# reonaledo/Multi-modality-Self-supervision

Measured on AMD Instinct MI355X. Metric: image-text pairs/sec pretraining step, BERT-base seq512, higher is better.
Workload: dtype f16

## Files before the change

### include/medvill_debug.h

```cpp
#ifndef MEDVILL_DEBUG_H_
#define MEDVILL_DEBUG_H_

#ifdef __cplusplus
extern "C" {
#endif

enum {
  MV_KNOB_ID_IMPL = 0,
  MV_KNOB_ID_GEMM_FORCE = 1,
  MV_KNOB_ID_GEMM_NJ = 2,
  MV_KNOB_ID_GEMM_DBG = 3,
  MV_KNOB_ID_ATTN_PLANES = 4,
  MV_KNOB_ID_PERSISTENT_CUS = 5,
  MV_KNOB_ID_ROWOPS_VARIANT = 6,
  MV_KNOB_ID_ATTN_FWD = 8,
  MV_KNOB_ID_GEMM_ROUNDS = 9,
  MV_KNOB_ID_ATTN_ORDER = 7
};
int mv_debug_set_knob(int id, int value);
int mv_debug_get_knob(int id);

#ifdef __cplusplus
}
#endif
#endif
```

### multi-modality-self-supervision_amd/_lib.py

```python
from __future__ import annotations

import ctypes as C
import os

import torch

HERE = os.path.dirname(os.path.abspath(__file__))
LIB_PATH = os.environ.get("MV_LIB_PATH") or os.path.join(HERE, "libmedvill_hip.so")
DBG_LIB_PATH = os.environ.get("MV_DBG_LIB_PATH") or (LIB_PATH[:-3] + "_dbg.so")

MV_F32, MV_BF16, MV_F16 = 0, 1, 2
EPI_NONE, EPI_BIAS, EPI_BIAS_GELU, EPI_BIAS_RES, EPI_DGELU, EPI_RES, EPI_BIAS_TANH, EPI_BIAS_GELU_D, EPI_MUL, EPI_BIAS_RELU, EPI_BIAS_RES_RELU = range(11)
_ERR = {-1: "MV_E_ARG (null pointer / bad size)", -2: "MV_E_SHAPE (unsupported shape or alignment)",
        -3: "MV_E_DTYPE", -4: "MV_E_WORKSPACE (workspace too small)", -5: "MV_E_NO_RCCL (librccl could not be loaded)"}

vp, i32, i64, f32, sz, u64, f64 = C.c_void_p, C.c_int, C.c_longlong, C.c_float, C.c_size_t, C.c_ulonglong, C.c_double

PROTOTYPES = {
    "mv_abi_version": [],
    "mv_build_info": [],
    "mv_stream_create_cumask": [vp, i32, C.POINTER(C.c_void_p)],
    "mv_stream_destroy": [vp],
    "mv_comm_unique_id": [vp],
    "mv_comm_init": [C.POINTER(C.c_void_p), i32, i32, vp],
# ... 53 lines not shown
    "mv_embed_rows": [i32, vp, vp, vp, vp, vp, vp, vp, vp, vp, i32, i32, i32, i32, i32, i32, f32, vp],
    "mv_ngram_ban": [vp, vp, i32, vp, vp, i32, i32, i32, vp, i32, vp, i32, vp, vp],
    "mv_logprob_topk_banned": [vp, i32, i32, i32, i32, i32, vp, i32, vp, vp, vp, vp, vp],
    "mv_bce_fwd_bwd": [vp, i32, vp, vp, i32, i32, vp, vp, i32, i32, vp, f32, vp, vp, vp, vp],
    "mv_rows_mul": [i32, vp, i32, vp, vp, i32, vp, i32, i32, vp, i32, vp],
    "mv_tensor_sqnorms": [vp, sz, vp, i32, vp, i32, vp, vp, vp],
    "mv_bce_multilabel": [vp, i32, vp, vp, i32, i32, vp, vp, i32, i32, vp, f32, vp, vp, vp, vp],
    "mv_bertadam_step": [vp, vp, vp, vp, vp, vp, sz, vp, i32, vp, i32, vp, f64, f64, f64, f32, f32, f32, i32, i32, f64, i32, vp, vp],
    "mv_lm_loss_fwd": [vp, i32, i32, i32, vp, vp, i32, f64, vp, vp, vp, vp],
    "mv_lm_loss_select": [vp, vp, vp, vp, i32, i32, i32, vp, vp, vp, vp],
    "mv_lm_loss_bwd": [vp, i32, i32, i32, vp, vp, vp, vp, i32, f64, vp, vp, vp, vp, vp, vp, i32, i32, vp],
    "mv_pair_draws": [u64, u64, i32, i32, vp, vp],
    "mv_pair_negatives": [vp, i32, i32, vp, u64, u64, vp, i32, vp, vp, vp],
    "mv_pair_assemble": [vp, vp, i32, vp, i32, i32, vp, vp, i32, i32, i32, i32, vp, vp, vp, vp, vp, vp, vp],
    "mv_rank_groups": [vp, vp, i32, i32, vp, i32, vp, vp, vp, vp, vp],
    "mv_report_draws": [u64, u64, i32, i32, vp, vp],
    "mv_report_assemble": [vp, vp, vp, i32, vp, i32, vp, vp, vp, i32, i32, i32, i32, i32, u64, u64, vp, vp, vp, vp, vp, vp, vp, vp, vp, vp],
    "mv_report_plan": [vp, vp, vp, vp, i32, i32, i32, i32, vp, vp, vp, vp, vp, vp, vp, vp],
    "mv_vqa_assemble": [vp, vp, vp, i32, vp, vp, vp, i32, vp, vp, i32, vp, i32, vp, vp, i32, i32, i32, i32, i32, vp, vp, vp, vp, vp, vp, vp, vp],
    "mv_vqa_score": [vp, vp, i32, i32, vp, vp, vp, i32, vp, vp, i32, vp, vp, vp],
    "mv_clf_assemble": [vp, vp, vp, vp, i32, vp, i32, vp, i32, vp, vp, i32, i32, i32, i32, i32, vp, vp, vp, vp, vp, vp, vp],
    "mv_clf_counts": [vp, i32, vp, i32, vp, i32, i32, vp, vp],
    "mv_bleu_words": [vp, i32, i32, i32, vp, vp, vp, i32, i64, i64, i64, vp, vp, vp],
    "mv_bleu_counts": [vp, i32, vp, i32, vp, i32, vp, i32, vp, vp, vp],
}
DEBUG_PROTOTYPES = {"mv_debug_set_knob": [i32, i32], "mv_debug_get_knob": [i32]}
_RESTYPE = {"mv_build_info": C.c_char_p, "mv_gemm_workspace_bytes": C.c_size_t, "mv_workspace_bytes": C.c_size_t,
            "mv_gemm_grouped_table_bytes": C.c_size_t, "mv_gemm_grouped_workspace_bytes": C.c_size_t}
ABI_VERSION = 6

KNOBS = {"impl": (0, 0), "gemm_force": (1, 0), "gemm_nj": (2, 0), "gemm_dbg": (3, 0), "attn_planes": (4, 16), "persistent_cus": (5, 0),
         "rowops_variant": (6, 0), "attn_order": (7, 0), "attn_fwd": (8, 0), "gemm_rounds": (9, 1)}

_lib = None
_dbg = None
_knobs = {k: d for k, (_, d) in KNOBS.items()}


def _open(path, protos):
    lib = C.CDLL(path)
    for name, args in protos.items():
        fn = getattr(lib, name)
        fn.argtypes = args
        fn.restype = _RESTYPE.get(name, C.c_int)
    if lib.mv_abi_version() != ABI_VERSION:
        raise RuntimeError(f"{path}: ABI version mismatch")
    return lib


def load(build_if_missing: bool = False):
    global _lib
    if _dbg is not None and any(_knobs[k] != d for k, (_, d) in KNOBS.items()):
        return _dbg
    if _lib is not None:
        return _lib
    if not os.path.exists(LIB_PATH):
        if build_if_missing:
            from ._build import build
            build()
        else:
            raise RuntimeError(
                f"{LIB_PATH} is missing: the gfx950 HIP extension has not been built. Run "
                "`python -c 'import __graft_entry__ as g; g.build()'` (needs hipcc). There is no fallback path.")
    _lib = _open(LIB_PATH, PROTOTYPES)
    return _lib


def set_knob(name: str, value: int):
    global _dbg
    kid, default = KNOBS[name]
    value = int(value)
    if _dbg is None:
        if value == default:
            return
        if not os.path.exists(DBG_LIB_PATH):
            raise RuntimeError(f"{DBG_LIB_PATH} is missing (the debug build of the library: __graft_entry__.build() makes both)")
        _dbg = _open(DBG_LIB_PATH, {**PROTOTYPES, **DEBUG_PROTOTYPES})
    check(_dbg.mv_debug_set_knob(kid, value), f"mv_debug_set_knob({name}, {value})")
    _knobs[name] = value


def get_knob(name: str) -> int:
    return _knobs[name]


def _knobs_from_env():
    spec = os.environ.get("MV_KNOBS", "")
    for item in filter(None, (x.strip() for x in spec.split(","))):
        k, _, v = item.partition("=")
        set_knob(k.strip(), int(v))


def check(rc: int, what: str):
    if rc == 0:
        return
    if rc <= -1000:
        raise RuntimeError(f"{what}: ncclResult_t {-1000 - rc}")
    if rc < 0:
        raise RuntimeError(f"{what}: {_ERR.get(rc, rc)}")
    raise RuntimeError(f"{what}: hipError_t {rc}")


def dt_of(t: torch.Tensor) -> int:
    if t.dtype == torch.float32:
        return MV_F32
    if t.dtype == torch.bfloat16:
        return MV_BF16
    if t.dtype == torch.float16:
        return MV_F16
    raise TypeError(f"unsupported dtype {t.dtype}")


def torch_dtype(dt: int):
    return {MV_F32: torch.float32, MV_BF16: torch.bfloat16, MV_F16: torch.float16}[dt]


# ... 16 lines not shown
```

### multi-modality-self-supervision_amd/csrc/mv_api.hip

```cpp
#include "mv_common.h"
#ifdef MV_DEBUG_KNOBS
#include "../../include/medvill_debug.h"
#endif

#define MV_KNOB_DEFAULTS {0, 0, 0, 0, 16, 0, 0, 0, 0, 1}
#ifdef MV_DEBUG_KNOBS
static int g_knobs[MV_KNOB_COUNT] = MV_KNOB_DEFAULTS;
int mv_knob(int id) { return g_knobs[id]; }
extern "C" int mv_debug_set_knob(int id, int value) {
  if (id < 0 || id >= MV_KNOB_COUNT) return MV_E_ARG;
  if (id == MV_KNOB_ATTN_PLANES && value != 8 && value != 12 && value != 16) return MV_E_ARG;
  g_knobs[id] = value;
  return MV_OK;
}
extern "C" int mv_debug_get_knob(int id) { return (id < 0 || id >= MV_KNOB_COUNT) ? MV_E_ARG : g_knobs[id]; }
#else
int mv_knob(int id) {
  static const int k[MV_KNOB_COUNT] = MV_KNOB_DEFAULTS;
  return k[id];
}
#endif

extern "C" int mv_abi_version(void) { return MV_ABI_VERSION; }
#ifdef MV_DEBUG_KNOBS
extern "C" const char* mv_build_info(void) { return "medvill-hip gfx950 debug-knobs (" __DATE__ " " __TIME__ ")"; }
#else
extern "C" const char* mv_build_info(void) { return "medvill-hip gfx950 (" __DATE__ " " __TIME__ ")"; }
#endif

extern "C" int mv_stream_create_cumask(const uint32_t* mask_words, int n_words, void** stream_out) {
  if (!mask_words || n_words <= 0 || !stream_out) return MV_E_ARG;
  hipStream_t st = nullptr;
  const hipError_t e = hipExtStreamCreateWithCUMask(&st, (uint32_t)n_words, mask_words);
  if (e != hipSuccess) return (int)e;
  *stream_out = (void*)st;
  return MV_OK;
}
extern "C" int mv_stream_destroy(void* stream) {
  if (!stream) return MV_E_ARG;
  const hipError_t e = hipStreamDestroy((hipStream_t)stream);
  return e == hipSuccess ? MV_OK : (int)e;
}
```

### multi-modality-self-supervision_amd/csrc/mv_attn.hip

```cpp
#include "mv_dispatch.h"

typedef float f32x2 __attribute__((ext_vector_type(2)));
#ifndef ATT_ABL
#define ATT_ABL 0
#endif
#ifndef ATT_EARLY_MASKS
#define ATT_EARLY_MASKS 0
#endif
#if ATT_ABL & 4096
__device__ unsigned long long g_att_prof[3][8];
__device__ unsigned long long g_att_tile[3][8];
#define PROF_DECL unsigned long long pt_ = clock64(), pacc_[6] = {0, 0, 0, 0, 0, 0}; unsigned long long ptile_[6] = {0, 0, 0, 0, 0, 0}
#define PROF_TILE_ARGS , unsigned long long (&ptile_)[6]
#define PROF_TILE_PASS , ptile_
#define PROF_T0 unsigned long long tt_ = clock64()
#define PROF_T(i, dep) do { asm volatile("s_nop 0" ::"v"(dep)); const unsigned long long n_ = clock64(); ptile_[i] += n_ - tt_; tt_ = n_; } while (0)
#define PROF_MARK(i) do { const unsigned long long n_ = clock64(); pacc_[i] += n_ - pt_; pt_ = n_; } while (0)
#define PROF_FLUSH(k) do { if (threadIdx.x == 0) { for (int i_ = 0; i_ < 6; ++i_) { atomicAdd(&g_att_prof[k][i_], pacc_[i_]); atomicAdd(&g_att_tile[k][i_], ptile_[i_]); } atomicAdd(&g_att_prof[k][7], 1ull); } } while (0)
#else
#define PROF_DECL
#define PROF_MARK(i)
#define PROF_FLUSH(k)
#define PROF_TILE_ARGS
#define PROF_TILE_PASS
// ... 187 lines not shown
      if (have == 0) { r = mv_hash32(base + ctr, k0, k1); ++ctr; have = PER; }
      const unsigned x = r & ((1u << SL) - 1u);
      r >>= SL;
      --have;
      if (x < lo) lt |= 1ull << l;
    }
  }
  out[w] = ~lt;
}

__device__ __forceinline__ int att_f(int r) { return (((r >> 1) & 1) << 2) | ((r >> 2) & 3); }
__device__ __forceinline__ int att_off(int r, int ch) { return r * 128 + ((ch ^ att_f(r)) << 4); }

__device__ __forceinline__ int acc_row(int reg, int h) { return (reg & 3) + 8 * (reg >> 2) + 4 * h; }

__device__ __forceinline__ void tile_load(u32x4 (&reg)[2], __amdgpu_buffer_rsrc_t rs, unsigned bytes, size_t rowbase,
                                          int row0, int nrows, int ld, int col0, int tid) {
#pragma unroll
  for (int i = 0; i < 2; ++i) {
    const int idx = tid + 256 * i;
    const int r = idx >> 3, ch = idx & 7;
    const bool ok = (row0 + r) < nrows;
    const unsigned off = (unsigned)(((rowbase + row0 + r) * (size_t)ld + col0 + ch * 8) * 2);
    reg[i] = __builtin_amdgcn_raw_buffer_load_b128(rs, ok ? off : bytes, 0, 0);
  }
}
__device__ __forceinline__ void tile_store(const u32x4 (&reg)[2], char* tile, int tid) {
#pragma unroll
  for (int i = 0; i < 2; ++i) {
    const int idx = tid + 256 * i;
    *(u32x4*)(tile + att_off(idx >> 3, idx & 7)) = reg[i];
  }
}
template <int NW>
__device__ __forceinline__ void tile_dma(dma_rsrc_t rs, unsigned bytes, size_t rowbase, int row0, int nrows, int ld,
                                         int col0, char* tile, int wid, int lane) {
#pragma unroll
  for (int i = 0; i < 8 / NW; ++i) {
    const int pc = wid + NW * i;
    const int r = pc * 8 + (lane >> 3), ch = (lane & 7) ^ att_f(r);
    const bool ok = (row0 + r) < nrows;
    const unsigned off = (unsigned)(((rowbase + row0 + r) * (size_t)ld + col0 + ch * 8) * 2);
    lds_dma16(rs, (MV_LDS void*)(tile + pc * 1024), ok ? off : bytes);
  }
}
#ifndef ATT_ISSUE_LATE
#define ATT_ISSUE_LATE 1
#endif
template <int N> __device__ __forceinline__ void att_wait_vmcnt() { asm volatile("s_waitcnt vmcnt(%0)" ::"n"(N) : "memory"); }
template <int PPW>
__device__ __forceinline__ void att_wait_stage(int younger) {
  if (younger <= 0) att_wait_vmcnt<0>();
  else if (younger == 1) att_wait_vmcnt<PPW>();
  else if (younger == 2) att_wait_vmcnt<2 * PPW>();
  else att_wait_vmcnt<3 * PPW>();
}

__device__ __forceinline__ bf16x8 frag_row(const char* tile, int base, int s, int l31, int h) {
  return *(const bf16x8*)(tile + att_off(base + l31, 2 * s + h));
}
__device__ __forceinline__ bf16x8 frag_tr(const char* tile, int cbase, int rb, int lane) {
  const int li = lane & 15, g = lane >> 4, h = g >> 1;
  const int col = cbase + 16 * (g & 1) + 4 * (li & 3);
  const int r = rb + 4 * h + (li >> 2);
  const int sub = (li & 1) * 8;
  bf16x4 lo = __builtin_amdgcn_ds_read_tr16_b64_v4bf16((MV_LDS bf16x4*)(tile + att_off(r, col >> 3) + sub));
  bf16x4 hi = __builtin_amdgcn_ds_read_tr16_b64_v4bf16((MV_LDS bf16x4*)(tile + att_off(r + 8, col >> 3) + sub));
  return __builtin_shufflevector(lo, hi, 0, 1, 2, 3, 4, 5, 6, 7);
}
struct FragLane { unsigned rk, tr; };
__device__ __forceinline__ FragLane frag_lane(int lane) {
// ... 345 lines not shown
        case 1: FWD_CALL(false, false); break;
        case 2: FWD_CALL(true, true); break;
        default: FWD_CALL(false, true); break;
      }
#undef FWD_CALL
    }
#if ATT_ABL & 4096
    asm volatile("s_nop 0" ::"v"(o[0][0]), "v"(o[1][15]));
#endif
    PROF_MARK(3);
    if (ATT_ISSUE_LATE && iss < nkt) issue();
    cur = next_tile(tmk.need, cur, nkt);
    ++done;
    PROF_MARK(4);
  }
  __builtin_amdgcn_s_barrier();
  const float ltot = lsum + __shfl_xor(lsum, 32, 64);
  const float inv = (a.drop_on ? a.inv_keep : 1.0f) / ltot;
  const int rows_ok = Lq - q0;
  char* patch = smem + wid * ATT_PATCH_BYTES;
  store_rows_tile<F16>(patch, o, inv, q_ok, a.out + (rowbase + q0) * (size_t)H + head * 64, (size_t)H, rows_ok, lane);
  if constexpr (F16) {
    if (a.out2) store_rows_tile<false>(patch, o, inv, q_ok, a.out2 + (rowbase + q0) * (size_t)H + head * 64, (size_t)H, rows_ok, lane);
  }
  if (q_ok && h == 0) a.lse[((size_t)b * a.A + head) * L + q] = (m2 + log2f(ltot)) * LN2;
#if ATT_ABL & 4096
  asm volatile("s_waitcnt vmcnt(0)");
#endif
  PROF_MARK(5);
  PROF_FLUSH(0);
}

template <bool MASKED, bool DROP, bool TAIL, bool F16>
__device__ __forceinline__ void dq_tile(const AttnArgs& a, unsigned tk, unsigned tv, unsigned tkt, const bf16x8 (&qf)[4], const bf16x8 (&dof)[4],
                                        f32x16 (&dq)[2], const uint32_t* myw, bool q_ok, int q, int b, int head, int k0, int Lv,
                                        float lse2, float dlt, float c2, int h, const unsigned long long* mp) {
  const float dlt_s = dlt * a.scale;
  const float dscale = DROP ? a.inv_keep * a.scale : a.scale;
#pragma unroll
  for (int kk = 0; kk < 2; ++kk) {
    f32x16 st, dp;
#pragma unroll
    for (int i = 0; i < 16; ++i) { st[i] = 0.f; dp[i] = 0.f; }
#pragma unroll
    for (int s = 0; s < 4; ++s) {
      st = mma32<F16>(frag_row_x(tk, 32 * kk, s), qf[s], st);
      dp = mma32<F16>(frag_row_x(tv, 32 * kk, s), dof[s], dp);
    }
    uint32_t w = 0xffffffffu;
    if (MASKED) { const int wi = (k0 >> 5) + kk; w = (q_ok && wi < a.W) ? myw[wi] : 0xffffffffu; }
    u64x8 m0, m1;
    if (DROP) sload_masks16(mp + 16 * kk, m0, m1);
#pragma unroll
    for (int r = 0; r < 16; ++r) {
      const int kr = acc_row(r, h);
      float pv;
      if (!MASKED) {
        pv = fexp2(fmaf(st[r], c2, -lse2));
      } else {
        const float v = fmaf(st[r], c2, ((w >> kr) & 1u) ? 0.f : MASK_ADD * LOG2E);
        pv = fexp2(v - lse2);
      }
      if (TAIL) pv = (k0 + 32 * kk + kr >= Lv) ? 0.f : pv;
      float t = fmaf(dp[r], dscale, -dlt_s);
      if (DROP) t = sel_set_else(t, -dlt_s, r < 8 ? m0[r & 7] : m1[r & 7]);
      st[r] = pv * t;
    }
#pragma unroll
    for (int s2 = 0; s2 < 2; ++s2) {
      const bf16x8 dsf = pack8t<F16>(st, s2);
#pragma unroll
      for (int dt = 0; dt < 2; ++dt)
        dq[dt] = mma32<F16>(frag_tr_x(tkt, dt, 32 * kk + 16 * s2), dsf, dq[dt]);
    }
  }
}

#define DQ_NS 4
template <bool F16>
__global__ __launch_bounds__(256, 2) void attn_bwd_dq_mfma_kernel(AttnArgs a) {
  extern __shared__ __attribute__((aligned(128))) char smem[];
  const int tid = threadIdx.x, lane = tid & 63, l31 = lane & 31, h = lane >> 5;
  const int wid = __builtin_amdgcn_readfirstlane(tid >> 6);
  int xb, head, b;
  att_block(a, xb, head, b);
  const int L = a.L, H = a.H, ld = 3 * a.H, T = a.T;
  const int qb0 = xb * 128, q0 = qb0 + wid * 32, q = q0 + l31;
  PROF_DECL;
  const TileMasks tmk = load_tile_masks_q(a.info, b, T, qb0 >> 6, min(q0 >> 6, T - 1), lane);
  const int Lv = a.cu ? a.cu[b + 1] - a.cu[b] : L;
  const int Lq = a.qlim ? min(Lv, a.qlim[b]) : Lv;
  if (qb0 >= Lv) return;
  const size_t rowbase = a.cu ? (size_t)a.cu[b] : (size_t)b * L;
  if (qb0 >= Lq) {
    const int r = qb0 + (tid >> 1);
    if (r < Lv) {
      bf16_t* z = a.dqkv + (rowbase + r) * (size_t)ld + head * 64 + 32 * (tid & 1);
#pragma unroll
      for (int c = 0; c < 32; c += 4) store4_16<F16>(z + c, 0.f, 0.f, 0.f, 0.f);
    }
    return;
  }
  const bool wave_on = q0 < Lq, q_ok = q < Lq;
  const size_t lrow = (size_t)b * L;
  __amdgpu_buffer_rsrc_t rs = __builtin_amdgcn_make_buffer_rsrc((void*)a.qkv, 0, a.bytes_qkv, 0x00020000);
  const dma_rsrc_t rsq = dma_rsrc(a.qkv, a.bytes_qkv);
  __amdgpu_buffer_rsrc_t rsd = __builtin_amdgcn_make_buffer_rsrc((void*)a.dctx, 0, a.bytes_ctx, 0x00020000);

  bf16x8 qf[4], dof[4];
#pragma unroll
  for (int s = 0; s < 4; ++s) {
    qf[s] = load_rowfrag_global(rs, a.bytes_qkv, rowbase + q, q_ok, ld, head * 64 + 16 * s + 8 * h);
    dof[s] = load_rowfrag_global(rsd, a.bytes_ctx, rowbase + q, q_ok, H, head * 64 + 16 * s + 8 * h);
  }
  const size_t sidx = ((size_t)b * a.A + head) * L + (q_ok ? q : 0);
  const float lse2 = q_ok ? a.lse_in[sidx] * LOG2E : INFINITY;
  float dlt = 0.f;
  {
    __amdgpu_buffer_rsrc_t rsc = __builtin_amdgcn_make_buffer_rsrc((void*)a.ctx, 0, a.bytes_ctx, 0x00020000);
#pragma unroll
    for (int s = 0; s < 4; ++s) {
      const bf16x8 of = load_rowfrag_global(rsc, a.bytes_ctx, rowbase + q, q_ok, H, head * 64 + 16 * s + 8 * h);
#pragma unroll
      for (int j = 0; j < 8; ++j) dlt = fmaf(frag_elem<F16>(of, j), frag_elem<F16>(dof[s], j), dlt);
    }
    dlt += __shfl_xor(dlt, 32, 64);
    if (q_ok && h == 0) a.delta_out[sidx] = dlt;
  }
  const float c2 = a.scale * LOG2E;
  f32x16 dq[2];
#pragma unroll
  for (int i = 0; i < 16; ++i) { dq[0][i] = 0.f; dq[1][i] = 0.f; }

  const int nkt = (Lv + 63) / 64;
  int cur = next_tile(tmk.need, -1, nkt);
  int iss = cur, issued = 0, done = 0;
  auto issue = [&]() {
    char* st_ = smem + (issued % DQ_NS) * 16384;
    tile_dma<4>(rsq, a.bytes_qkv, rowbase, iss * 64, Lv, ld, H + head * 64, st_, wid, lane);
    tile_dma<4>(rsq, a.bytes_qkv, rowbase, iss * 64, Lv, ld, 2 * H + head * 64, st_ + 8192, wid, lane);
    ++issued;
    iss = next_tile(tmk.need, iss, nkt);
  };
#pragma unroll
  for (int i = 0; i < DQ_NS - 1; ++i)
    if (iss < nkt) issue();
  const uint32_t* myw = a.bits + (lrow + (q_ok ? q : 0)) * a.W;
  const FragLane fl = frag_lane(lane);
  const unsigned smem_a = lds_addr(smem);
  PROF_MARK(0);
  while (cur < nkt) {
    att_wait_stage<4>(issued - done - 1);
    PROF_MARK(1);
    __builtin_amdgcn_s_barrier();
    PROF_MARK(2);
    __builtin_amdgcn_sched_barrier(0);
    if (!ATT_ISSUE_LATE && iss < nkt) issue();
    const unsigned tKa = smem_a + (unsigned)(done % DQ_NS) * 16384u;
    const int cls = !wave_on ? 0 : (((tmk.w_is1 >> cur) & 1) ? 1 : (((tmk.w_nz >> cur) & 1) ? 2 : 0));
    if (wave_on && cls != 0) {
      const int k0 = cur * 64;
      const bool tail = (k0 + 64 > Lv);
      unsigned rk_ = fl.rk, tr_ = fl.tr;
      int h_ = h;
      asm volatile("" : "+v"(rk_), "+v"(tr_), "+v"(h_));
      const unsigned tk = tKa + rk_, tv = tKa + 8192u + rk_, tkt = tKa + tr_;
      const unsigned long long* mp = a.drop_on ? (const unsigned long long*)a.dropbits + dbits_block(a, (size_t)b * a.A + head, q0 >> 5, cur) : nullptr;
      const int variant = (cls == 1 ? 0 : 1) | (tail ? 2 : 0) | (a.drop_on ? 4 : 0);
#define DQ_CALL(M_, D_, T_) dq_tile<M_, D_, T_, F16>(a, tk, tv, tkt, qf, dof, dq, myw, q_ok, q, b, head, k0, Lv, lse2, dlt, c2, h_, mp)
      switch (variant) {
        case 0: DQ_CALL(false, false, false); break;
        case 1: DQ_CALL(true, false, false); break;
        case 2: case 3: DQ_CALL(true, false, true); break;
        case 4: DQ_CALL(false, true, false); break;
        case 5: DQ_CALL(true, true, false); break;
        default: DQ_CALL(true, true, true); break;
      }
#undef DQ_CALL
    }
#if ATT_ABL & 4096
    asm volatile("s_nop 0" ::"v"(dq[0][0]), "v"(dq[1][15]));
#endif
    PROF_MARK(3);
    if (ATT_ISSUE_LATE && iss < nkt) issue();
    cur = next_tile(tmk.need, cur, nkt);
    ++done;
    PROF_MARK(4);
  }
  __builtin_amdgcn_s_barrier();
  store_rows_tile<F16>(smem + wid * ATT_PATCH_BYTES, dq, 1.0f, q_ok, a.dqkv + (rowbase + q0) * (size_t)ld + head * 64, (size_t)ld, Lv - q0,
                       lane);
#if ATT_ABL & 4096
  asm volatile("s_waitcnt vmcnt(0)");
#endif
  PROF_MARK(5);
  PROF_FLUSH(1);
}

#define KV_STAGE (8192 + 8192 + 256 + 256 + 1024 + 1024)
static_assert(KV_STAGE % 128 == 0 && ATT_PATCH_BYTES % 128 == 0, "frag_row_x / frag_tr_x XOR bits 4-6 of (tile base + lane word): every tile base must be a multiple of 128 bytes");
template <bool MASKED, bool DROP, bool F16>
__device__ __forceinline__ void dkv_tile(const AttnArgs& a, const char* tQ, const char* tD, const float* s_lse, const float* s_dl,
                                         const uint32_t* s_w, const bf16x8 (&kf)[4], const bf16x8 (&vf)[4], f32x16 (&dk)[2],
                                         f32x16 (&dv)[2], int b, int head, int cur, int key, int wid, float c2, int lane_in, const uint32_t* s_db,
                                         const FragLane& fl) {
  int lane = lane_in;
  unsigned rk_ = fl.rk, tr_ = fl.tr;
  asm volatile("" : "+v"(lane), "+v"(rk_), "+v"(tr_));
  const int l31 = lane & 31, h = lane >> 5;
  const unsigned tq = lds_addr(tQ) + rk_, td = lds_addr(tD) + rk_, tqt = lds_addr(tQ) + tr_, tdt = lds_addr(tD) + tr_;
  const float dscale = DROP ? a.inv_keep * a.scale : a.scale;
#pragma unroll
  for (int qq = 0; qq < 2; ++qq) {
    f32x16 sc, dp;
#pragma unroll
    for (int i = 0; i < 16; ++i) { sc[i] = 0.f; dp[i] = 0.f; }
    {
// ... 651 lines not shown
                           const int32_t* cu, int total_rows, const int32_t* qlim, void* stream_) {
  hipStream_t stream = (hipStream_t)stream_;
  if (!qkv || !bits || !tileinfo || !ctx || !lse || B <= 0 || L <= 0 || A <= 0 || dh <= 0) return MV_E_ARG;
  if (!mv_dtype_ok(dtype)) return MV_E_DTYPE;
  if (ctx_bf16 && dtype != MV_F16) return MV_E_DTYPE;
  const int rcd = dropbits_check(p_drop, dropbits, B, L, A);
  if (rcd) return rcd;
  const int H = A * dh;
  if (mv_is16(dtype) && g_mv_impl == 0) {
    if (dh != 64) return MV_E_SHAPE;
    if (cu && (total_rows <= 0 || total_rows > B * L)) return MV_E_ARG;
    const size_t nrow = cu ? (size_t)total_rows : (size_t)B * L;
    const size_t bq = nrow * 3 * H * 2;
    if (bq >= 0x7fffffffULL || (((uintptr_t)qkv) & 15) || (((uintptr_t)ctx) & 7) || (((uintptr_t)ctx_bf16) & 7)) return MV_E_SHAPE;
    AttnArgs a = attn_args(qkv, bits, tileinfo, B, L, A, dh, bq, p_drop, dropbits, cu, qlim);
    a.out = (bf16_t*)ctx; a.out2 = (bf16_t*)ctx_bf16; a.lse = lse;
    static bool attr = false;
    if (!attr) {
      (void)hipFuncSetAttribute((const void*)attn_fwd_mfma_kernel<false>, hipFuncAttributeMaxDynamicSharedMemorySize, FWD_NS * 16384);
      (void)hipFuncSetAttribute((const void*)attn_fwd_mfma_kernel<true>, hipFuncAttributeMaxDynamicSharedMemorySize, FWD_NS * 16384);
      attr = true;
    }
    return mv_with_type(dtype, MfmaAccept{}, [&](auto t) -> int {
      hipLaunchKernelGGL(attn_fwd_mfma_kernel<decltype(t)::code == MV_F16>, dim3((L + 127) / 128, A, B), dim3(256), FWD_NS * 16384, stream, a);
      return (int)hipGetLastError();
    });
  }
  if (dh > 128 || cu || qlim) return MV_E_SHAPE;
  int rc = mv_with_type(dtype, [&](auto t) { return launch_simple_fwd<MV_T(t)>(qkv, bits, ctx, lse, B, L, A, dh, p_drop, dropbits, stream); });
  if (rc == MV_OK && ctx_bf16) rc = mv_cast(ctx, MV_F16, ctx_bf16, MV_BF16, (size_t)B * L * H, stream_);
  return rc;
}

template <typename T>
static int launch_simple_bwd(const void* qkv, const void* ctx, const void* dctx, const float* lse, const uint32_t* bits,
                             void* dqkv, float* delta, int B, int L, int A, int dh, float p_drop, const uint32_t* dropbits, hipStream_t stream) {
  SArgs<T> s{};
  s.dropbits = p_drop > 0.f ? (const unsigned long long*)dropbits : nullptr; s.inv_keep = attn_inv_keep(p_drop);
  s.NQB = (L + 31) / 32; s.NKT = (L + 63) / 64;
  s.qkv = (const T*)qkv; s.ctx = (const T*)ctx; s.dctx = (const T*)dctx; s.dqkv = (T*)dqkv; s.bits = bits;
  s.lse_in = lse; s.delta = delta;
  s.B = B; s.L = L; s.A = A; s.H = A * dh; s.W = (L + 31) / 32; s.dh = dh; s.scale = 1.0f / sqrtf((float)dh);
  const long long waves = (long long)B * A * L;
  const unsigned blocks = (unsigned)((waves + 3) / 4);
  hipLaunchKernelGGL(attn_delta_kernel<T>, dim3(blocks), dim3(256), 0, stream, s.ctx, s.dctx, delta, B, L, A, s.H, dh);
  MV_CHECK_LAUNCH();
  hipLaunchKernelGGL(attn_bwd_dq_simple_kernel<T>, dim3(blocks), dim3(256), 0, stream, s);
  MV_CHECK_LAUNCH();
  hipLaunchKernelGGL(attn_bwd_dkv_simple_kernel<T>, dim3(blocks), dim3(256), 0, stream, s);
  MV_CHECK_LAUNCH();
  return MV_OK;
}

extern "C" int mv_attn_bwd(int dtype, const void* qkv, const void* ctx, const void* dctx, const float* lse, const uint32_t* bits,
                           const uint8_t* tileinfo, void* dqkv, float* delta, int B, int L, int A, int dh, float p_drop,
                           const uint32_t* dropbits, const int32_t* cu, int total_rows, const int32_t* qlim, void* stream_) {
  hipStream_t stream = (hipStream_t)stream_;
  if (!qkv || !ctx || !dctx || !lse || !bits || !tileinfo || !dqkv || !delta || B <= 0 || L <= 0 || A <= 0 || dh <= 0)
    return MV_E_ARG;
  if (!mv_dtype_ok(dtype)) return MV_E_DTYPE;
  const int rcd = dropbits_check(p_drop, dropbits, B, L, A);
  if (rcd) return rcd;
  const int H = A * dh;
  if (mv_is16(dtype) && g_mv_impl == 0) {
    if (dh != 64) return MV_E_SHAPE;
    if (cu && (total_rows <= 0 || total_rows > B * L)) return MV_E_ARG;
    const size_t nrow = cu ? (size_t)total_rows : (size_t)B * L;
    const size_t bq = nrow * 3 * H * 2, bc = nrow * H * 2;
    if (bq >= 0x7fffffffULL || (((uintptr_t)qkv) & 15) || (((uintptr_t)dctx) & 15) || (((uintptr_t)dqkv) & 7)) return MV_E_SHAPE;
    AttnArgs a = attn_args(qkv, bits, tileinfo, B, L, A, dh, bq, p_drop, dropbits, cu, qlim);
    a.ctx = (const bf16_t*)ctx; a.dctx = (const bf16_t*)dctx; a.dqkv = (bf16_t*)dqkv;
    a.lse_in = lse; a.delta = delta; a.delta_out = delta;
    a.bytes_ctx = (unsigned)bc;
    a.bytes_stat = (unsigned)((size_t)B * A * L * 4); a.bytes_bits = (unsigned)((size_t)B * L * a.W * 4);
    static bool attr = false;
    if (!attr) {
      (void)hipFuncSetAttribute((const void*)attn_bwd_dq_mfma_kernel<false>, hipFuncAttributeMaxDynamicSharedMemorySize, DQ_NS * 16384);
      (void)hipFuncSetAttribute((const void*)attn_bwd_dkv_mfma_kernel<false>, hipFuncAttributeMaxDynamicSharedMemorySize, DKV_NS * KV_STAGE);
      (void)hipFuncSetAttribute((const void*)attn_bwd_dq_mfma_kernel<true>, hipFuncAttributeMaxDynamicSharedMemorySize, DQ_NS * 16384);
      (void)hipFuncSetAttribute((const void*)attn_bwd_dkv_mfma_kernel<true>, hipFuncAttributeMaxDynamicSharedMemorySize, DKV_NS * KV_STAGE);
      attr = true;
    }
    dim3 grid((L + 127) / 128, A, B);
    return mv_with_type(dtype, MfmaAccept{}, [&](auto t) -> int {
      hipLaunchKernelGGL(attn_bwd_dq_mfma_kernel<decltype(t)::code == MV_F16>, grid, dim3(256), DQ_NS * 16384, stream, a);
      MV_CHECK_LAUNCH();
      hipLaunchKernelGGL(attn_bwd_dkv_mfma_kernel<decltype(t)::code == MV_F16>, grid, dim3(256), DKV_NS * KV_STAGE, stream, a);
      return (int)hipGetLastError();
    });
  }
  if (dh > 128 || cu || qlim) return MV_E_SHAPE;
  return mv_with_type(dtype, [&](auto t) {
    return launch_simple_bwd<MV_T(t)>(qkv, ctx, dctx, lse, bits, dqkv, delta, B, L, A, dh, p_drop, dropbits, stream);
  });
}

template <typename T, typename TO>
static int launch_simple_probs(const void* qkv, const uint32_t* bits, const float* lse, void* probs, int B, int L, int A, int dh, float p_drop,
                               const uint32_t* dropbits, int head_mean, hipStream_t stream) {
  PSArgs<T> s{};
  s.dropbits = p_drop > 0.f ? (const unsigned long long*)dropbits : nullptr; s.inv_keep = attn_inv_keep(p_drop);
  s.NQB = (L + 31) / 32; s.NKT = (L + 63) / 64;
  s.qkv = (const T*)qkv; s.bits = bits; s.lse = lse; s.out = probs; s.head_mean = head_mean ? 1 : 0;
  s.B = B; s.L = L; s.A = A; s.H = A * dh; s.W = (L + 31) / 32; s.dh = dh; s.scale = 1.0f / sqrtf((float)dh);
  const long long waves = (long long)B * (head_mean ? 1 : A) * L;
  hipLaunchKernelGGL((attn_probs_simple_kernel<T, TO>), dim3((unsigned)((waves + 3) / 4)), dim3(256), 0, stream, s);
  MV_CHECK_LAUNCH();
  return MV_OK;
}

extern "C" int mv_attn_probs(int dtype, const void* qkv, const uint32_t* bits, const uint8_t* tileinfo, const float* lse, void* probs,
                             int out_dtype, int B, int L, int A, int dh, float p_drop, const uint32_t* dropbits, int head_mean, void* stream_) {
  typedef mv_pairs<mv_pair<float, float>, mv_pair<bf16_t, float>, mv_pair<bf16_t, bf16_t>, mv_pair<f16_t, float>, mv_pair<f16_t, f16_t>> Accept;
  hipStream_t stream = (hipStream_t)stream_;
  if (!qkv || !bits || !tileinfo || !lse || !probs || B <= 0 || L <= 0 || A <= 0 || dh <= 0) return MV_E_ARG;
  if (!mv_dtype_ok(dtype)) return MV_E_DTYPE;
  if (out_dtype != MV_F32 && out_dtype != dtype) return MV_E_ARG;
  const int Tt = (L + 63) / 64;
// ... 33 lines not shown
```

### multi-modality-self-supervision_amd/csrc/mv_common.h

```cpp
#pragma once
#include <hip/hip_runtime.h>
#include <stdint.h>
#include <math.h>
#include "../../include/medvill.h"

typedef __bf16 bf16_t;
typedef __attribute__((ext_vector_type(8))) __bf16 bf16x8;
typedef __attribute__((ext_vector_type(4))) __bf16 bf16x4;
typedef __attribute__((ext_vector_type(2))) __bf16 bf16x2;
typedef __attribute__((ext_vector_type(4))) float f32x4;
typedef __attribute__((ext_vector_type(16))) float f32x16;
typedef __attribute__((ext_vector_type(4))) unsigned u32x4;
typedef __attribute__((ext_vector_type(2))) unsigned u32x2;
typedef _Float16 f16_t;
typedef __attribute__((ext_vector_type(8))) _Float16 f16x8;
typedef __attribute__((ext_vector_type(4))) _Float16 f16x4;

#define MV_LDS __attribute__((address_space(3)))

enum {
  MV_KNOB_IMPL = 0,
  MV_KNOB_GEMM_FORCE = 1,
  MV_KNOB_GEMM_NJ = 2,
  MV_KNOB_GEMM_DBG = 3,
  MV_KNOB_ATTN_PLANES = 4,
  MV_KNOB_PERSISTENT_CUS = 5,
  MV_KNOB_ROWOPS_VARIANT = 6,
  MV_KNOB_ATTN_ORDER = 7,
  MV_KNOB_ATTN_FWD = 8,
  MV_KNOB_GEMM_ROUNDS = 9,
  MV_KNOB_COUNT = 10
};
__attribute__((visibility("hidden"))) int mv_knob(int id);
#define g_mv_impl (mv_knob(MV_KNOB_IMPL))

#define MV_CHECK_LAUNCH()                           \
  do {                                              \
    hipError_t e__ = hipGetLastError();             \
    if (e__ != hipSuccess) return (int)e__;         \
  } while (0)

__device__ __forceinline__ float bf2f(bf16_t x) { return (float)x; }
__device__ __forceinline__ bf16_t f2bf(float x) { return (bf16_t)x; }

template <typename T> __device__ __forceinline__ float ldf(const T* p);
template <> __device__ __forceinline__ float ldf<float>(const float* p) { return *p; }
template <> __device__ __forceinline__ float ldf<bf16_t>(const bf16_t* p) { return (float)*p; }
template <> __device__ __forceinline__ float ldf<f16_t>(const f16_t* p) { return (float)*p; }
template <typename T> __device__ __forceinline__ void stf(T* p, float v);
template <> __device__ __forceinline__ void stf<float>(float* p, float v) { *p = v; }
template <> __device__ __forceinline__ void stf<bf16_t>(bf16_t* p, float v) { *p = (bf16_t)v; }
template <> __device__ __forceinline__ void stf<f16_t>(f16_t* p, float v) { *p = (f16_t)v; }

template <typename T> __device__ __forceinline__ f32x4 ld4(const T* p);
template <> __device__ __forceinline__ f32x4 ld4<float>(const float* p) { return *(const f32x4*)p; }
template <> __device__ __forceinline__ f32x4 ld4<bf16_t>(const bf16_t* p) {
  bf16x4 v = *(const bf16x4*)p;
  f32x4 r = {(float)v[0], (float)v[1], (float)v[2], (float)v[3]};
  return r;
}
template <> __device__ __forceinline__ f32x4 ld4<f16_t>(const f16_t* p) {
  f16x4 v = *(const f16x4*)p;
  f32x4 r = {(float)v[0], (float)v[1], (float)v[2], (float)v[3]};
  return r;
}
template <typename T> __device__ __forceinline__ void st4(T* p, f32x4 v);
template <> __device__ __forceinline__ void st4<float>(float* p, f32x4 v) { *(f32x4*)p = v; }
// ... 135 lines not shown
```

### multi-modality-self-supervision_amd/hip_ops.py

```python
from __future__ import annotations

import ctypes

import torch

from . import _lib as L
from ._lib import (EPI_BIAS, EPI_BIAS_GELU, EPI_BIAS_GELU_D, EPI_BIAS_RELU, EPI_BIAS_RES, EPI_BIAS_RES_RELU, EPI_BIAS_TANH, EPI_DGELU,
                   EPI_MUL, EPI_NONE, EPI_RES, MV_BF16, MV_F16,
                   MV_F32)


def _lib():
    return L.load()


def gemm(a, b, c, *, ta=False, tb=False, M, N, K, lda=None, ldb=None, ldc=None, bias=None, epi=EPI_NONE, r=None, ldr=None,
         c2=None, ldc2=None, c3=None, ldc3=None, splitk=1, ws=None, accumulate=False, p_drop=0.0, drop_key=0, alpha=None, colsum_part=None):
    L.require_cuda(a, b, c, bias, r, c2, c3, ws, alpha, colsum_part)
    if colsum_part is not None and (colsum_part.dtype != torch.float32 or colsum_part.numel() < 2 * ((M + 255) // 256) * N):
        raise ValueError("colsum_part: f32 [2*ceil(M/256), N]")
    lda = lda if lda is not None else (M if ta else K)
    ldb = ldb if ldb is not None else (N if tb else K)
    ldc = ldc if ldc is not None else N
    ldr = ldr if ldr is not None else N
# ... 344 lines not shown


def set_impl(impl: int):
    L.set_knob("impl", 1 if impl else 0)


def get_impl() -> int:
    return L.get_knob("impl")


def set_attn_planes(planes: int):
    L.set_knob("attn_planes", planes if planes in (8, 12) else 16)


def attn_drop_prob(p_drop: float) -> float:
    n = L.get_knob("attn_planes")
    return round(p_drop * (1 << n)) / float(1 << n)


def set_rowops_variant(v: int = 0):
    L.set_knob("rowops_variant", v)


def set_gemm_rounds(on: int = 1):
    L.set_knob("gemm_rounds", 1 if on else 0)


def set_attn_fwd(variant: int = 0):
    L.set_knob("attn_fwd", variant)


def set_attn_order(order: int = 0):
    L.set_knob("attn_order", order)


class RcclComm:

    def __init__(self, rank: int, world: int, unique_id: bytes):
        import ctypes
        if len(unique_id) != 128:
            raise ValueError("unique_id: 128 bytes (RcclComm.unique_id() on rank 0)")
        self._h = ctypes.c_void_p()
        buf = ctypes.create_string_buffer(bytes(unique_id), 128)
        L.check(_lib().mv_comm_init(ctypes.byref(self._h), int(rank), int(world), buf), "mv_comm_init")
        self.rank, self.world = rank, world

    @staticmethod
    def unique_id() -> bytes:
        import ctypes
        buf = ctypes.create_string_buffer(128)
        L.check(_lib().mv_comm_unique_id(buf), "mv_comm_unique_id")
        return buf.raw

    def allreduce_async(self, t, stream=None):
        L.require_cuda(t)
        if not t.is_contiguous():
            raise ValueError("allreduce_async: contiguous tensor")
        st = (stream or torch.cuda.current_stream()).cuda_stream
        L.check(_lib().mv_comm_allreduce_async(self._h, L.ptr(t), t.numel(), L.dt_of(t), st), "mv_comm_allreduce_async")

    def wait(self, stream=None):
        st = (stream or torch.cuda.current_stream()).cuda_stream
        L.check(_lib().mv_comm_wait(self._h, st), "mv_comm_wait")

    def destroy(self):
        if self._h:
# ... 649 lines not shown
```

Baseline: 2843.

## Shrink dQ backward LDS ring to two stages and raise occupancy to three blocks

The attention dQ backward kernel now splits each 64-key K/V tile into two 32-row half stages and double-buffers them, which halves dynamic LDS from 64KB to 32KB. Launch bounds go from 2 to 3 blocks per CU so more waves can hide latency. The inner tile routine is split into per-half calls with adjusted mask and tail offsets. The prefetch depth drops from three tiles in flight to two, so memory latency hiding within a block is shallower in exchange for more resident blocks. A debug occupancy query is also added.

```diff
diff --git a/include/medvill_debug.h b/include/medvill_debug.h
--- a/include/medvill_debug.h
+++ b/include/medvill_debug.h
@@ -17,6 +17,11 @@
   MV_KNOB_ID_GEMM_ROUNDS = 9,
   MV_KNOB_ID_ATTN_ORDER = 7
 };
+enum {
+  MV_QUERY_ID_ATTN_OCC_FWD = 64,
+  MV_QUERY_ID_ATTN_OCC_DQ = 65,
+  MV_QUERY_ID_ATTN_OCC_DKV = 66
+};
 int mv_debug_set_knob(int id, int value);
 int mv_debug_get_knob(int id);
 
diff --git a/multi-modality-self-supervision_amd/_lib.py b/multi-modality-self-supervision_amd/_lib.py
--- a/multi-modality-self-supervision_amd/_lib.py
+++ b/multi-modality-self-supervision_amd/_lib.py
@@ -109,6 +109,8 @@
 KNOBS = {"impl": (0, 0), "gemm_force": (1, 0), "gemm_nj": (2, 0), "gemm_dbg": (3, 0), "attn_planes": (4, 16), "persistent_cus": (5, 0),
          "rowops_variant": (6, 0), "attn_order": (7, 0), "attn_fwd": (8, 0), "gemm_rounds": (9, 1)}
 
+QUERIES = {"attn_occ_fwd": 64, "attn_occ_dq": 65, "attn_occ_dkv": 66}
+
 _lib = None
 _dbg = None
 _knobs = {k: d for k, (_, d) in KNOBS.items()}
@@ -143,22 +145,34 @@
     return _lib
 
 
-def set_knob(name: str, value: int):
+def _load_dbg():
     global _dbg
-    kid, default = KNOBS[name]
-    value = int(value)
     if _dbg is None:
-        if value == default:
-            return
         if not os.path.exists(DBG_LIB_PATH):
             raise RuntimeError(f"{DBG_LIB_PATH} is missing (the debug build of the library: __graft_entry__.build() makes both)")
         _dbg = _open(DBG_LIB_PATH, {**PROTOTYPES, **DEBUG_PROTOTYPES})
+    return _dbg
+
+
+def set_knob(name: str, value: int):
+    kid, default = KNOBS[name]
+    value = int(value)
+    if _dbg is None and value == default:
+        return
+    _load_dbg()
     check(_dbg.mv_debug_set_knob(kid, value), f"mv_debug_set_knob({name}, {value})")
     _knobs[name] = value
 
 
 def get_knob(name: str) -> int:
     return _knobs[name]
+
+
+def query(name: str) -> int:
+    v = _load_dbg().mv_debug_get_knob(QUERIES[name])
+    if v < 0:
+        raise RuntimeError(f"mv_debug_get_knob({name}): hipError_t {-v}")
+    return v
 
 
 def _knobs_from_env():
diff --git a/multi-modality-self-supervision_amd/csrc/mv_api.hip b/multi-modality-self-supervision_amd/csrc/mv_api.hip
--- a/multi-modality-self-supervision_amd/csrc/mv_api.hip
+++ b/multi-modality-self-supervision_amd/csrc/mv_api.hip
@@ -13,7 +13,10 @@
   g_knobs[id] = value;
   return MV_OK;
 }
-extern "C" int mv_debug_get_knob(int id) { return (id < 0 || id >= MV_KNOB_COUNT) ? MV_E_ARG : g_knobs[id]; }
+extern "C" int mv_debug_get_knob(int id) {
+  if (id >= MV_QUERY_ATTN_OCC_FWD && id <= MV_QUERY_ATTN_OCC_DKV) return mv_attn_occupancy(id);
+  return (id < 0 || id >= MV_KNOB_COUNT) ? MV_E_ARG : g_knobs[id];
+}
 #else
 int mv_knob(int id) {
   static const int k[MV_KNOB_COUNT] = MV_KNOB_DEFAULTS;
diff --git a/multi-modality-self-supervision_amd/csrc/mv_attn.hip b/multi-modality-self-supervision_amd/csrc/mv_attn.hip
--- a/multi-modality-self-supervision_amd/csrc/mv_attn.hip
+++ b/multi-modality-self-supervision_amd/csrc/mv_attn.hip
@@ -243,11 +243,11 @@
     *(u32x4*)(tile + att_off(idx >> 3, idx & 7)) = reg[i];
   }
 }
-template <int NW>
+template <int NW, int PIECES = 8>
 __device__ __forceinline__ void tile_dma(dma_rsrc_t rs, unsigned bytes, size_t rowbase, int row0, int nrows, int ld,
                                          int col0, char* tile, int wid, int lane) {
 #pragma unroll
-  for (int i = 0; i < 8 / NW; ++i) {
+  for (int i = 0; i < PIECES / NW; ++i) {
     const int pc = wid + NW * i;
     const int r = pc * 8 + (lane >> 3), ch = (lane & 7) ^ att_f(r);
     const bool ok = (row0 + r) < nrows;
@@ -659,36 +659,36 @@
 }
 
 template <bool MASKED, bool DROP, bool TAIL, bool F16>
-__device__ __forceinline__ void dq_tile(const AttnArgs& a, unsigned tk, unsigned tv, unsigned tkt, const bf16x8 (&qf)[4], const bf16x8 (&dof)[4],
-                                        f32x16 (&dq)[2], const uint32_t* myw, bool q_ok, int q, int b, int head, int k0, int Lv,
+__device__ __forceinline__ void dq_half(const AttnArgs& a, unsigned tk, unsigned tv, unsigned tkt, const bf16x8 (&qf)[4], const bf16x8 (&dof)[4],
+                                        f32x16 (&dq)[2], const uint32_t* myw, bool q_ok, int k0, int kk, int Lv,
                                         float lse2, float dlt, float c2, int h, const unsigned long long* mp) {
   const float dlt_s = dlt * a.scale;
   const float dscale = DROP ? a.inv_keep * a.scale : a.scale;
-#pragma unroll
-  for (int kk = 0; kk < 2; ++kk) {
+  {
     f32x16 st, dp;
 #pragma unroll
     for (int i = 0; i < 16; ++i) { st[i] = 0.f; dp[i] = 0.f; }
 #pragma unroll
     for (int s = 0; s < 4; ++s) {
-      st = mma32<F16>(frag_row_x(tk, 32 * kk, s), qf[s], st);
-      dp = mma32<F16>(frag_row_x(tv, 32 * kk, s), dof[s], dp);
-    }
-    uint32_t w = 0xffffffffu;
-    if (MASKED) { const int wi = (k0 >> 5) + kk; w = (q_ok && wi < a.W) ? myw[wi] : 0xffffffffu; }
+      st = mma32<F16>(frag_row_x(tk, 0, s), qf[s], st);
+      dp = mma32<F16>(frag_row_x(tv, 0, s), dof[s], dp);
+    }
+    uint32_t wh = 0xffffffffu;
+    if (MASKED) { const int wi = (k0 >> 5) + kk; wh = ((q_ok && wi < a.W) ? myw[wi] : 0xffffffffu) >> (4 * h); }
+    const int klim = Lv - k0 - 32 * kk - 4 * h;
     u64x8 m0, m1;
     if (DROP) sload_masks16(mp + 16 * kk, m0, m1);
 #pragma unroll
     for (int r = 0; r < 16; ++r) {
-      const int kr = acc_row(r, h);
+      const int kr0 = acc_row(r, 0);
       float pv;
       if (!MASKED) {
         pv = fexp2(fmaf(st[r], c2, -lse2));
       } else {
-        const float v = fmaf(st[r], c2, ((w >> kr) & 1u) ? 0.f : MASK_ADD * LOG2E);
+        const float v = fmaf(st[r], c2, ((wh >> kr0) & 1u) ? 0.f : MASK_ADD * LOG2E);
         pv = fexp2(v - lse2);
       }
-      if (TAIL) pv = (k0 + 32 * kk + kr >= Lv) ? 0.f : pv;
+      if (TAIL) pv = (kr0 >= klim) ? 0.f : pv;
       float t = fmaf(dp[r], dscale, -dlt_s);
       if (DROP) t = sel_set_else(t, -dlt_s, r < 8 ? m0[r & 7] : m1[r & 7]);
       st[r] = pv * t;
@@ -698,14 +698,16 @@
       const bf16x8 dsf = pack8t<F16>(st, s2);
 #pragma unroll
       for (int dt = 0; dt < 2; ++dt)
-        dq[dt] = mma32<F16>(frag_tr_x(tkt, dt, 32 * kk + 16 * s2), dsf, dq[dt]);
+        dq[dt] = mma32<F16>(frag_tr_x(tkt, dt, 16 * s2), dsf, dq[dt]);
     }
   }
 }
 
 #define DQ_NS 4
+#define DQ_STAGE 8192
+static_assert(DQ_STAGE % 128 == 0 && 4 * ATT_PATCH_BYTES <= DQ_NS * DQ_STAGE, "the epilogue's four row patches reuse the ring");
 template <bool F16>
-__global__ __launch_bounds__(256, 2) void attn_bwd_dq_mfma_kernel(AttnArgs a) {
+__global__ __launch_bounds__(256, 3) void attn_bwd_dq_mfma_kernel(AttnArgs a) {
   extern __shared__ __attribute__((aligned(128))) char smem[];
   const int tid = threadIdx.x, lane = tid & 63, l31 = lane & 31, h = lane >> 5;
   const int wid = __builtin_amdgcn_readfirstlane(tid >> 6);
@@ -763,14 +765,17 @@
   int cur = next_tile(tmk.need, -1, nkt);
   int iss = cur, issued = 0, done = 0;
   auto issue = [&]() {
-    char* st_ = smem + (issued % DQ_NS) * 16384;
-    tile_dma<4>(rsq, a.bytes_qkv, rowbase, iss * 64, Lv, ld, H + head * 64, st_, wid, lane);
-    tile_dma<4>(rsq, a.bytes_qkv, rowbase, iss * 64, Lv, ld, 2 * H + head * 64, st_ + 8192, wid, lane);
+    char* st_ = smem + (issued & 1) * (2 * DQ_STAGE);
+#pragma unroll
+    for (int kk = 0; kk < 2; ++kk) {
+      tile_dma<4, 4>(rsq, a.bytes_qkv, rowbase, iss * 64 + 32 * kk, Lv, ld, H + head * 64, st_ + kk * DQ_STAGE, wid, lane);
+      tile_dma<4, 4>(rsq, a.bytes_qkv, rowbase, iss * 64 + 32 * kk, Lv, ld, 2 * H + head * 64, st_ + kk * DQ_STAGE + 4096, wid, lane);
+    }
     ++issued;
     iss = next_tile(tmk.need, iss, nkt);
   };
 #pragma unroll
-  for (int i = 0; i < DQ_NS - 1; ++i)
+  for (int i = 0; i < DQ_NS / 2; ++i)
     if (iss < nkt) issue();
   const uint32_t* myw = a.bits + (lrow + (q_ok ? q : 0)) * a.W;
   const FragLane fl = frag_lane(lane);
@@ -782,8 +787,8 @@
     __builtin_amdgcn_s_barrier();
     PROF_MARK(2);
     __builtin_amdgcn_sched_barrier(0);
-    if (!ATT_ISSUE_LATE && iss < nkt) issue();
-    const unsigned tKa = smem_a + (unsigned)(done % DQ_NS) * 16384u;
+    if (done > 0 && iss < nkt) issue();
+    const unsigned tKa = smem_a + (unsigned)(done & 1) * (unsigned)(2 * DQ_STAGE);
     const int cls = !wave_on ? 0 : (((tmk.w_is1 >> cur) & 1) ? 1 : (((tmk.w_nz >> cur) & 1) ? 2 : 0));
     if (wave_on && cls != 0) {
       const int k0 = cur * 64;
@@ -791,10 +796,12 @@
       unsigned rk_ = fl.rk, tr_ = fl.tr;
       int h_ = h;
       asm volatile("" : "+v"(rk_), "+v"(tr_), "+v"(h_));
-      const unsigned tk = tKa + rk_, tv = tKa + 8192u + rk_, tkt = tKa + tr_;
+      const unsigned tk = tKa + rk_, tv = tKa + 4096u + rk_, tkt = tKa + tr_;
       const unsigned long long* mp = a.drop_on ? (const unsigned long long*)a.dropbits + dbits_block(a, (size_t)b * a.A + head, q0 >> 5, cur) : nullptr;
       const int variant = (cls == 1 ? 0 : 1) | (tail ? 2 : 0) | (a.drop_on ? 4 : 0);
-#define DQ_CALL(M_, D_, T_) dq_tile<M_, D_, T_, F16>(a, tk, tv, tkt, qf, dof, dq, myw, q_ok, q, b, head, k0, Lv, lse2, dlt, c2, h_, mp)
+#define DQ_CALL(M_, D_, T_)                                                                                      \
+  dq_half<M_, D_, T_, F16>(a, tk, tv, tkt, qf, dof, dq, myw, q_ok, k0, 0, Lv, lse2, dlt, c2, h_, mp);            \
+  dq_half<M_, D_, T_, F16>(a, tk + DQ_STAGE, tv + DQ_STAGE, tkt + DQ_STAGE, qf, dof, dq, myw, q_ok, k0, 1, Lv, lse2, dlt, c2, h_, mp)
       switch (variant) {
         case 0: DQ_CALL(false, false, false); break;
         case 1: DQ_CALL(true, false, false); break;
@@ -809,7 +816,6 @@
     asm volatile("s_nop 0" ::"v"(dq[0][0]), "v"(dq[1][15]));
 #endif
     PROF_MARK(3);
-    if (ATT_ISSUE_LATE && iss < nkt) issue();
     cur = next_tile(tmk.need, cur, nkt);
     ++done;
     PROF_MARK(4);
@@ -1527,6 +1533,24 @@
   return rc;
 }
 
+template <typename K>
+static int attn_occ_of(K kern, size_t lds) {
+  int n = 0;
+  hipError_t e = hipFuncSetAttribute((const void*)kern, hipFuncAttributeMaxDynamicSharedMemorySize, (int)lds);
+  if (e == hipSuccess) e = hipOccupancyMaxActiveBlocksPerMultiprocessor(&n, kern, 256, lds);
+  return e == hipSuccess ? n : -(int)e;
+}
+int mv_attn_occupancy(int query) {
+  int a, b;
+  switch (query) {
+    case MV_QUERY_ATTN_OCC_FWD: a = attn_occ_of(attn_fwd_mfma_kernel<false>, FWD_NS * 16384); b = attn_occ_of(attn_fwd_mfma_kernel<true>, FWD_NS * 16384); break;
+    case MV_QUERY_ATTN_OCC_DQ: a = attn_occ_of(attn_bwd_dq_mfma_kernel<false>, DQ_NS * DQ_STAGE); b = attn_occ_of(attn_bwd_dq_mfma_kernel<true>, DQ_NS * DQ_STAGE); break;
+    case MV_QUERY_ATTN_OCC_DKV: a = attn_occ_of(attn_bwd_dkv_mfma_kernel<false>, DKV_NS * KV_STAGE); b = attn_occ_of(attn_bwd_dkv_mfma_kernel<true>, DKV_NS * KV_STAGE); break;
+    default: return MV_E_ARG;
+  }
+  return a < b ? a : b;
+}
+
 template <typename T>
 static int launch_simple_bwd(const void* qkv, const void* ctx, const void* dctx, const float* lse, const uint32_t* bits,
                              void* dqkv, float* delta, int B, int L, int A, int dh, float p_drop, const uint32_t* dropbits, hipStream_t stream) {
@@ -1570,15 +1594,15 @@
     a.bytes_stat = (unsigned)((size_t)B * A * L * 4); a.bytes_bits = (unsigned)((size_t)B * L * a.W * 4);
     static bool attr = false;
     if (!attr) {
-      (void)hipFuncSetAttribute((const void*)attn_bwd_dq_mfma_kernel<false>, hipFuncAttributeMaxDynamicSharedMemorySize, DQ_NS * 16384);
+      (void)hipFuncSetAttribute((const void*)attn_bwd_dq_mfma_kernel<false>, hipFuncAttributeMaxDynamicSharedMemorySize, DQ_NS * DQ_STAGE);
       (void)hipFuncSetAttribute((const void*)attn_bwd_dkv_mfma_kernel<false>, hipFuncAttributeMaxDynamicSharedMemorySize, DKV_NS * KV_STAGE);
-      (void)hipFuncSetAttribute((const void*)attn_bwd_dq_mfma_kernel<true>, hipFuncAttributeMaxDynamicSharedMemorySize, DQ_NS * 16384);
+      (void)hipFuncSetAttribute((const void*)attn_bwd_dq_mfma_kernel<true>, hipFuncAttributeMaxDynamicSharedMemorySize, DQ_NS * DQ_STAGE);
       (void)hipFuncSetAttribute((const void*)attn_bwd_dkv_mfma_kernel<true>, hipFuncAttributeMaxDynamicSharedMemorySize, DKV_NS * KV_STAGE);
       attr = true;
     }
     dim3 grid((L + 127) / 128, A, B);
     return mv_with_type(dtype, MfmaAccept{}, [&](auto t) -> int {
-      hipLaunchKernelGGL(attn_bwd_dq_mfma_kernel<decltype(t)::code == MV_F16>, grid, dim3(256), DQ_NS * 16384, stream, a);
+      hipLaunchKernelGGL(attn_bwd_dq_mfma_kernel<decltype(t)::code == MV_F16>, grid, dim3(256), DQ_NS * DQ_STAGE, stream, a);
       MV_CHECK_LAUNCH();
       hipLaunchKernelGGL(attn_bwd_dkv_mfma_kernel<decltype(t)::code == MV_F16>, grid, dim3(256), DKV_NS * KV_STAGE, stream, a);
       return (int)hipGetLastError();
diff --git a/multi-modality-self-supervision_amd/csrc/mv_common.h b/multi-modality-self-supervision_amd/csrc/mv_common.h
--- a/multi-modality-self-supervision_amd/csrc/mv_common.h
+++ b/multi-modality-self-supervision_amd/csrc/mv_common.h
@@ -33,6 +33,8 @@
 };
 __attribute__((visibility("hidden"))) int mv_knob(int id);
 #define g_mv_impl (mv_knob(MV_KNOB_IMPL))
+enum { MV_QUERY_ATTN_OCC_FWD = 64, MV_QUERY_ATTN_OCC_DQ = 65, MV_QUERY_ATTN_OCC_DKV = 66 };
+__attribute__((visibility("hidden"))) int mv_attn_occupancy(int query);
 
 #define MV_CHECK_LAUNCH()                           \
   do {                                              \
diff --git a/multi-modality-self-supervision_amd/hip_ops.py b/multi-modality-self-supervision_amd/hip_ops.py
--- a/multi-modality-self-supervision_amd/hip_ops.py
+++ b/multi-modality-self-supervision_amd/hip_ops.py
@@ -400,6 +400,10 @@
 
 def set_attn_order(order: int = 0):
     L.set_knob("attn_order", order)
+
+
+def attn_occupancy() -> dict:
+    return {k: L.query("attn_occ_" + k) for k in ("fwd", "dq", "dkv")}
 
 
 class RcclComm:
```

New measurement: 2866 (median of 6 runs). No clear change (+0.8%).
